# ldkong1205/OpenESS

Hardware: AMD Instinct MI355X
Metric: event-frames/sec fwd+bwd @640x480 B=8 (higher is better)
Workload: dtype bf16; 1 GPU; DSEC 640x480 5-bin x20 voxelizer + frame2voxel_pixel_distill pre-train step (E2VID-recurrent encoder x20, SemSegE2VID decoder, dilated-R50 teacher, Dice+CE), batch 8/GPU, random-init weights; global_batch=8, parallelism=dp1

## Files before the change

### openess_amd/csrc/conv5x5s2_halo.h

```cpp
constexpr int S2_PH = 8, S2_PW = 16;
constexpr int S2_HH = 2 * S2_PH + 3, S2_XW = 18;
constexpr int S2_BLOCKS = 2 * S2_HH * S2_XW;
constexpr int S2_HINSTR = (S2_BLOCKS + 63) / 64;
constexpr int S2_HALO_BYTES = S2_HINSTR * 4 * 1024;
constexpr int S2_SLAB = 64 * 64;
constexpr int S2_RING_PLAIN = 6, S2_RING_FUSED = 5;
constexpr int S2_LDS = S2_HALO_BYTES + S2_RING_PLAIN * S2_SLAB;
constexpr int S2_VH = S2_HH + 4, S2_VW = 2 * S2_PW + 3 + 4;
constexpr int S2_VINSTR = (S2_VH * S2_VW + 255) / 256;
constexpr int S2_VTOTAL = (S2_VH * S2_VW + 63) / 64;
constexpr int S2_VOX_BYTES = S2_VTOTAL * 1024;
constexpr int S2_LDS_FUSED = S2_HALO_BYTES + S2_RING_FUSED * S2_SLAB + S2_VOX_BYTES;
struct S2Head {
    const uint16_t* x8;
    long long x8_stride;
    const uint16_t* hw;
    const float* hb;
    int relu;
    const float* ev;
    int Ctot, c0, Cs, normalize;
    const double* stats;
};
constexpr int S2_IMG_PITCH = 72;

template <typename F, int... Is>
__device__ __forceinline__ void s2_for_taps(F&& f, std::integer_sequence<int, Is...>) { (f(std::integral_constant<int, Is>{}), ...); }

template <bool FUSED>
__device__ __forceinline__ void conv5x5s2_halo_tile(const ConvArgs& a, const S2Head& hd, const int bid, unsigned char* smem) {
    constexpr int S2_RING = FUSED ? S2_RING_FUSED : S2_RING_PLAIN;
    const int tile_n = bid % a.tiles_n;
    int patch = bid / a.tiles_n;
    const int tiles_x = (a.Wo + S2_PW - 1) / S2_PW, tiles_y = (a.Ho + S2_PH - 1) / S2_PH;
    const int ox0 = (patch % tiles_x) * S2_PW; patch /= tiles_x;
    const int oy0 = (patch % tiles_y) * S2_PH;
    const int b = patch / tiles_y;
    const int n0 = tile_n * 64;
    const int tid = threadIdx.x, lane = tid & 63;
    const int wave = __builtin_amdgcn_readfirstlane(tid >> 6);
    const int wm = wave >> 1, wn = wave & 1;
    constexpr int MT = 2, NT = 1;
    const int nchunks = a.Cin >> 5;
    const int NS = nchunks * 25;

    const long long in_bytes = FUSED ? (((long long)a.B * a.H * a.W - 1) * hd.x8_stride + 8) * 2
                                     : (((long long)a.B * a.H * a.W - 1) * a.in_pix_stride + a.Cin) * 2;
    __amdgpu_buffer_rsrc_t rsA = __builtin_amdgcn_make_buffer_rsrc(FUSED ? (void*)hd.x8 : (void*)a.in, 0, (FUSED && !hd.x8) ? 0 : (int)in_bytes, 0x00020000);
    __amdgpu_buffer_rsrc_t rsB = __builtin_amdgcn_make_buffer_rsrc((void*)a.w, 0, 0x7ffffff0, 0x00020000);

    unsigned hoff[FUSED ? 1 : S2_HINSTR];
#pragma unroll
    for (int i = 0; i < (FUSED ? 0 : S2_HINSTR); ++i) {
        const int u = (wave * S2_HINSTR + i) * 16 + (lane >> 2), slot = lane & 3;
        const int p = u / (S2_HH * S2_XW), rem = u - p * (S2_HH * S2_XW);
        const int hy = rem / S2_XW, xi = rem - hy * S2_XW;
        const int hx = 2 * xi + p;
        const int f = ((xi >> 2) & 1) | (((hy >> 1) & 1) << 1);
        const int iy = 2 * oy0 - 2 + hy, ix = 2 * ox0 - 2 + hx;
        const bool ok = u < S2_BLOCKS && hx < 2 * S2_PW + 3 && (unsigned)iy < (unsigned)a.H && (unsigned)ix < (unsigned)a.W;
        hoff[i] = ok ? (unsigned)((((long long)b * a.H + iy) * a.W + ix) * a.in_pix_stride * 2 + ((slot ^ f) << 4)) : 0x80000000u;
    }
    unsigned boff;
    {
        const int row = wave * 16 + (lane >> 2), slot = lane & 3;
        boff = (unsigned)(((n0 + row) * a.Kpad + ((slot ^ ((row >> 2) & 3)) << 3)) * 2);
    }
    auto issue_halo = [&](int cc) {
#pragma unroll
        for (int i = 0; i < (FUSED ? 0 : S2_HINSTR); ++i) {
            const unsigned voff = hoff[i] == 0x80000000u ? 0x80000000u : hoff[i] + (unsigned)(cc * 64);
            __builtin_amdgcn_raw_ptr_buffer_load_lds(rsA, (__attribute__((address_space(3))) void*)(smem + (wave * S2_HINSTR + i) * 1024),
                                                     16, voff, 0, 0, 0);
        }
    };
    auto issue_w = [&](int s, int buf) {
        const int cc = s / 25, tap = s - cc * 25;
        const unsigned voff = s < NS ? boff + (unsigned)((tap * a.Cin + cc * 32) * 2) : 0x80000000u;
        __builtin_amdgcn_raw_ptr_buffer_load_lds(rsB, (__attribute__((address_space(3))) void*)(smem + S2_HALO_BYTES + buf * S2_SLAB + wave * 1024),
                                                 16, voff, 0, 0, 0);
    };

    f32x16_t acc[2];
#pragma unroll
    for (int i = 0; i < 2; ++i)
#pragma unroll
        for (int e = 0; e < 16; ++e) acc[i][e] = 0.0f;

    const uint32_t lds0 = (uint32_t)(uintptr_t)smem;
    const int r31 = lane & 31, half = lane >> 5;
    const int a_px = (r31 & 7) + 8 * (r31 >> 4);
    uint32_t va[2][3][2], vb;
#pragma unroll
    for (int i = 0; i < 2; ++i) {
        const int py = 4 * wm + 2 * i + ((r31 >> 3) & 1);
#pragma unroll
        for (int sv = 0; sv < 3; ++sv)
#pragma unroll
            for (int rp = 0; rp < 2; ++rp) {
                const int f = (((a_px + sv) >> 2) & 1) | (((py + rp) & 1) << 1);
                va[i][sv][rp] = lds0 + (uint32_t)((2 * py * S2_XW + a_px) * 64 + ((half ^ f) << 4));
            }
    }
    {
        const int n = wn * 32 + r31;
        vb = lds0 + (uint32_t)(S2_HALO_BYTES + n * 64 + ((half ^ ((n >> 2) & 3)) << 4));
    }

#define S2_READ(FA, FB, R_, S_, KS_, BUF_)                                                                              \
    {                                                                                                                   \
        constexpr int blk_ = ((((S_) & 1) * S2_HH + (R_)) * S2_XW + ((S_) >> 1)) * 64;                                   \
        _Pragma("unroll") for (int i = 0; i < 2; ++i)                                                                   \
            asm volatile("ds_read_b128 %0, %1 offset:%2" : "=v"(FA[i]) : "v"(va[i][(S_) >> 1][((R_) >> 1) & 1] ^ (uint32_t)((KS_) << 5)), "n"(blk_) : "memory"); \
        asm volatile("ds_read_b128 %0, %1" : "=v"(FB[0]) : "v"((vb ^ (uint32_t)((KS_) << 5)) + (uint32_t)((BUF_) * S2_SLAB)) : "memory");  \
    }
#define S2_MMA(FA, FB)                                                                                                  \
    {                                                                                                                   \
        _Pragma("unroll") for (int i = 0; i < 2; ++i)                                                                   \
            acc[i] = __builtin_amdgcn_mfma_f32_32x32x16_bf16(FB[0], FA[i], acc[i], 0, 0, 0);                            \
    }

    if constexpr (FUSED) {
        unsigned char* vox = smem + S2_HALO_BYTES + S2_RING_FUSED * S2_SLAB;
        bf16x8_t wf[13];
        {
            const int p32 = lane & 31, hi = lane >> 5;
#pragma unroll
            for (int ks = 0; ks < 13; ++ks) wf[ks] = *reinterpret_cast<const bf16x8_t*>(hd.hw + (size_t)p32 * 256 + (ks * 2 + hi) * 8);
        }
        if (hd.ev) {
#pragma unroll
            for (int s = 0; s < S2_RING - 1; ++s) issue_w(s, s);
            const double nnz = hd.stats ? hd.stats[2] : 0.0;
            const bool active = hd.normalize && nnz > 0.0;
            float mean = 0.f, stdv = 1.f;
            if (active) {
                const float nf = (float)nnz;
                mean = (float)hd.stats[0] / nf;
                stdv = sqrtf(__fsub_rn((float)hd.stats[1] / nf, __fmul_rn(mean, mean)));
            }
            const long long hw_ = (long long)a.H * a.W;
            float raw[4][5];
            bool okv[4];
#pragma unroll
            for (int i = 0; i < 4; ++i) {
                const int v = tid + 256 * i;
                const int vy = v / S2_VW, vx = v - vy * S2_VW;
                const int iy = 2 * oy0 - 4 + vy, ix = 2 * ox0 - 4 + vx;
                okv[i] = v < S2_VH * S2_VW && (unsigned)iy < (unsigned)a.H && (unsigned)ix < (unsigned)a.W;
                const float* src = hd.ev + ((long long)b * hd.Ctot + hd.c0) * hw_ + (long long)iy * a.W + ix;
#pragma unroll
                for (int c = 0; c < 5; ++c) raw[i][c] = (okv[i] && c < hd.Cs) ? src[c * hw_] : 0.0f;
            }
#pragma unroll
            for (int i = 0; i < 4; ++i) {
                const int v = tid + 256 * i;
                float f[8] = {0.f, 0.f, 0.f, 0.f, 0.f, 0.f, 0.f, 0.f};
#pragma unroll
                for (int c = 0; c < 5; ++c) {
                    float q = raw[i][c];
                    if (active) q = __fmul_rn((q != 0.0f) ? 1.0f : 0.0f, __fsub_rn(q, mean)) / stdv;
                    f[c] = (okv[i] && c < hd.Cs) ? q : 0.0f;
                }
                const u32x4_t o = {pack_bf16x2(f[0], f[1]), pack_bf16x2(f[2], f[3]), pack_bf16x2(f[4], f[5]), pack_bf16x2(f[6], f[7])};
                if (v < S2_VTOTAL * 64)
                    asm volatile("ds_write_b128 %0, %1" :: "v"((uint32_t)(uintptr_t)vox + (uint32_t)(v * 16)), "v"(o) : "memory");
            }
            asm volatile("s_waitcnt lgkmcnt(0)" ::: "memory");
        } else {
#pragma unroll
            for (int i = 0; i < S2_VINSTR; ++i) {
                const int v = (wave * S2_VINSTR + i) * 64 + lane;
                const int vy = v / S2_VW, vx = v - vy * S2_VW;
                const int iy = 2 * oy0 - 4 + vy, ix = 2 * ox0 - 4 + vx;
                const bool ok = v < S2_VH * S2_VW && (unsigned)iy < (unsigned)a.H && (unsigned)ix < (unsigned)a.W;
                const unsigned voff = ok ? (unsigned)((((long long)b * a.H + iy) * a.W + ix) * hd.x8_stride * 2) : 0x80000000u;
                if (wave * S2_VINSTR + i < S2_VTOTAL)
                    __builtin_amdgcn_raw_ptr_buffer_load_lds(rsA, (__attribute__((address_space(3))) void*)(vox + (wave * S2_VINSTR + i) * 1024), 16, voff, 0, 0, 0);
            }
#pragma unroll
            for (int s = 0; s < S2_RING - 1; ++s) issue_w(s, s);
        }
        float bq[4][4];
#pragma unroll
        for (int q = 0; q < 4; ++q)
#pragma unroll
            for (int k = 0; k < 4; ++k) bq[q][k] = hd.hb ? hd.hb[8 * q + 4 * (lane >> 5) + k] : 0.0f;
        asm volatile("s_waitcnt vmcnt(0)" ::: "memory");
        __builtin_amdgcn_s_barrier();
        const uint32_t vox0 = (uint32_t)(uintptr_t)vox, pl0 = (uint32_t)(uintptr_t)smem;
        const int hi = lane >> 5;
        static_assert(((S2_BLOCKS + 31) / 32) % 2 == 0, "M-tiles are taken in pairs");
        for (int pr = wave; pr < (S2_BLOCKS + 31) / 64; pr += 4) {
            int uu_[2], hy_[2], xi_[2];
            bool inside_[2];
            uint32_t vbase[2];
#pragma unroll
            for (int z = 0; z < 2; ++z) {
                const int u = (2 * pr + z) * 32 + (lane & 31);
                uu_[z] = u;
                const int uu = u < S2_BLOCKS ? u : 0;
                const int p = uu / (S2_HH * S2_XW), rem = uu - p * (S2_HH * S2_XW);
                const int hy = rem / S2_XW, xi = rem - hy * S2_XW;
                int hx = 2 * xi + p;
                inside_[z] = u < S2_BLOCKS && hx < 2 * S2_PW + 3 && (unsigned)(2 * oy0 - 2 + hy) < (unsigned)a.H &&
                             (unsigned)(2 * ox0 - 2 + hx) < (unsigned)a.W;
                hx = hx < 2 * S2_PW + 3 ? hx : 0;
                hy_[z] = hy; xi_[z] = xi;
                vbase[z] = vox0 + (uint32_t)((hy * S2_VW + hx) * 16);
            }
            f32x16_t hacc[2];
#pragma unroll
            for (int z = 0; z < 2; ++z)
#pragma unroll
                for (int e = 0; e < 16; ++e) hacc[z][e] = 0.0f;
            bf16x8_t pa[2], pb[2];
#define S2_HREAD(DST, KS_)                                                                                             \
            {                                                                                                         \
                constexpr int t0_ = 2 * (KS_), t1_ = 2 * (KS_) + 1 < 25 ? 2 * (KS_) + 1 : 0;                            \
                const uint32_t off_ = hi ? (uint32_t)(((t1_ / 5) * S2_VW + t1_ % 5) * 16) : (uint32_t)(((t0_ / 5) * S2_VW + t0_ % 5) * 16); \
                asm volatile("ds_read_b128 %0, %1" : "=v"(DST[0]) : "v"(vbase[0] + off_) : "memory");                  \
                asm volatile("ds_read_b128 %0, %1" : "=v"(DST[1]) : "v"(vbase[1] + off_) : "memory");                  \
            }
            S2_HREAD(pa, 0)
            s2_for_taps([&](auto kc) __attribute__((always_inline)) {
                constexpr int ks = decltype(kc)::value;
                if constexpr (ks + 1 < 13) {
                    if constexpr (ks & 1) { S2_HREAD(pa, ks + 1) } else { S2_HREAD(pb, ks + 1) }
                    if constexpr (ks & 1) asm volatile("s_waitcnt lgkmcnt(2)" : "+v"(pb[0]), "+v"(pb[1]) :: "memory");
                    else asm volatile("s_waitcnt lgkmcnt(2)" : "+v"(pa[0]), "+v"(pa[1]) :: "memory");
                } else {
                    if constexpr (ks & 1) asm volatile("s_waitcnt lgkmcnt(0)" : "+v"(pb[0]), "+v"(pb[1]) :: "memory");
                    else asm volatile("s_waitcnt lgkmcnt(0)" : "+v"(pa[0]), "+v"(pa[1]) :: "memory");
                }
#pragma unroll
                for (int z = 0; z < 2; ++z)
                    hacc[z] = __builtin_amdgcn_mfma_f32_32x32x16_bf16(wf[ks], (ks & 1) ? pb[z] : pa[z], hacc[z], 0, 0, 0);
            }, std::make_integer_sequence<int, 13>{});
#undef S2_HREAD
#pragma unroll
            for (int z = 0; z < 2; ++z) {
                if (uu_[z] >= S2_BLOCKS) continue;
                const uint32_t f = (uint32_t)(((xi_[z] >> 2) & 1) | (((hy_[z] >> 1) & 1) << 1));
#pragma unroll
                for (int q = 0; q < 4; ++q) {
                    float v[4];
#pragma unroll
                    for (int k = 0; k < 4; ++k) {
                        v[k] = hacc[z][q * 4 + k] + bq[q][k];
                        if (hd.relu) v[k] = fmaxf(v[k], 0.0f);
                        v[k] = inside_[z] ? v[k] : 0.0f;
                    }
                    const uint2 o = make_uint2(pack_bf16x2(v[0], v[1]), pack_bf16x2(v[2], v[3]));
                    asm volatile("ds_write_b64 %0, %1" :: "v"(pl0 + (uint32_t)(uu_[z] * 64) + (((uint32_t)q ^ f) << 4) + (uint32_t)(8 * hi)), "v"(o) : "memory");
                }
            }
        }
        asm volatile("s_waitcnt lgkmcnt(0)" ::: "memory");
    } else {
#pragma unroll
        for (int s = 0; s < S2_RING - 1; ++s) issue_w(s, s);
    }
    int sg = 0, buf = 0;
    for (int cc = 0; cc < nchunks; ++cc) {
        if (cc > 0) __builtin_amdgcn_s_barrier();
        issue_halo(cc);
        asm volatile("s_waitcnt vmcnt(0)" ::: "memory");
        __builtin_amdgcn_s_barrier();
        bf16x8_t fa0[MT], fb0[NT], fa1[MT], fb1[NT];
        S2_READ(fa0, fb0, 0, 0, 0, buf)
        s2_for_taps([&](auto tc) __attribute__((always_inline)) {
            constexpr int t = decltype(tc)::value, r = t / 5, s = t - r * 5;
            if (t > 0) {
                asm volatile("s_waitcnt vmcnt(%0)" :: "n"(S2_RING - 3) : "memory");
                __builtin_amdgcn_s_barrier();
            }
            const int nb = buf + 1 == S2_RING ? 0 : buf + 1;
            issue_w(sg + S2_RING - 1, buf == 0 ? S2_RING - 1 : buf - 1);
            __builtin_amdgcn_s_setprio(3);
            S2_READ(fa1, fb1, r, s, 1, buf)
            OESS_FRAG_WAIT(3, fa0, fb0)
            S2_MMA(fa0, fb0)
            if constexpr (t < 24) {
                constexpr int r2 = (t + 1) / 5, s2 = (t + 1) - r2 * 5;
                S2_READ(fa0, fb0, r2, s2, 0, nb)
                OESS_FRAG_WAIT(3, fa1, fb1)
            } else {
                OESS_FRAG_WAIT(0, fa1, fb1)
            }
            S2_MMA(fa1, fb1)
            __builtin_amdgcn_s_setprio(0);
            ++sg; buf = nb;
        }, std::make_integer_sequence<int, 25>{});
    }
#undef S2_READ
#undef S2_MMA
    asm volatile("s_waitcnt vmcnt(0)" ::: "memory");
    __syncthreads();

    uint16_t* img = reinterpret_cast<uint16_t*>(smem);
    {
        float bq[4][4];
#pragma unroll
        for (int q = 0; q < 4; ++q)
#pragma unroll
            for (int k = 0; k < 4; ++k) bq[q][k] = a.bias ? a.bias[n0 + wn * 32 + 8 * q + 4 * half + k] : 0.0f;
#pragma unroll
        for (int i = 0; i < 2; ++i) {
            const int py = 4 * wm + 2 * i + ((r31 >> 3) & 1);
            uint16_t* dst = img + (py * S2_PW + a_px) * S2_IMG_PITCH + wn * 32 + 4 * half;
#pragma unroll
            for (int q = 0; q < 4; ++q) {
                float v[4];
#pragma unroll
                for (int k = 0; k < 4; ++k) {
                    v[k] = acc[i][q * 4 + k] + bq[q][k];
                    if (a.relu) v[k] = fmaxf(v[k], 0.0f);
                }
                uint2 o;
                o.x = pack_bf16x2(v[0], v[1]);
                o.y = pack_bf16x2(v[2], v[3]);
                *reinterpret_cast<uint2*>(dst + 8 * q) = o;
            }
        }
    }
    __syncthreads();
#pragma unroll
    for (int k = 0; k < 4; ++k) {
        const int idx = tid + k * 256, pl = idx >> 3, c = idx & 7;
        const int oy = oy0 + (pl >> 4), ox = ox0 + (pl & 15);
        if (oy < a.Ho && ox < a.Wo)
            out_store16(a.out + (((long long)b * a.Ho + oy) * a.Wo + ox) * a.out_pix_stride + n0 + c * 8,
                        *reinterpret_cast<const uint4*>(img + pl * S2_IMG_PITCH + c * 8));
    }
}

template <bool FUSED>
__global__ __launch_bounds__(256, 2) void conv5x5s2_halo_kernel(ConvArgs a, S2Head hd) {
    extern __shared__ __attribute__((aligned(16))) unsigned char smem[];
    const int nwg = a.tiles_m * a.tiles_n;
    int bid = blockIdx.x;
    {
        const int q = nwg >> 3, r = nwg & 7, xcd = bid & 7, idx = bid >> 3;
        bid = (xcd < r ? xcd * (q + 1) : r * (q + 1) + (xcd - r) * q) + idx;
    }
    conv5x5s2_halo_tile<FUSED>(a, hd, bid, smem);
}

struct S2Group {
    ConvArgs a[2];
    int start8[3];
};
__global__ __launch_bounds__(256, 2) void conv5x5s2_halo_group_kernel(S2Group g) {
    extern __shared__ __attribute__((aligned(16))) unsigned char smem[];
    const int xcd = blockIdx.x & 7, idx = blockIdx.x >> 3;
    const int p = idx >= g.start8[1] ? 1 : 0;
    const int li = idx - g.start8[p];
    const ConvArgs& a = g.a[p];
    const int nwg = a.tiles_m * a.tiles_n;
    const int q = nwg >> 3, r = nwg & 7;
    if (li >= q + (xcd < r ? 1 : 0)) return;
    conv5x5s2_halo_tile<false>(a, S2Head{}, (xcd < r ? xcd * (q + 1) : r * (q + 1) + (xcd - r) * q) + li, smem);
}
```

### openess_amd/csrc/conv_fwd.hip

```cpp
#include <hip/hip_runtime.h>
#include <stdint.h>
#include <stdlib.h>
#include <string.h>
#include <stdio.h>
#include <map>
#include <mutex>
#include <vector>
#include "oess.h"
#include "oess_common.h"

namespace {
#include <type_traits>
#include <utility>
using namespace oess;

#include "conv_args.h"
#include "conv_frag.h"
#include "conv_general.h"
#include "conv_dma.h"
#include "conv3x3_halo.h"
#pragma clang diagnostic push
#pragma clang diagnostic ignored "-Wunused-lambda-capture"
#include "conv_lstm_w128.h"
#include "conv_w128_gemm.h"
// ... 376 lines not shown
}

int oess_conv2d_fwd_route(int B, int H, int W, int Cin, int Cout, int R, int S, int stride, int pad, int dil, int has_bias,
                          int relu, int has_residual, int out_is_f32, int with_tile_stats, long long in_pix_stride,
                          long long out_pix_stride, long long res_pix_stride, int out_aligned16, size_t workspace_bytes) {
    ConvPlan p;
    const int rc = conv_plan(conv_call(B, H, W, Cin, Cout, R, S, stride, pad, dil, relu, has_bias, has_residual, out_is_f32, with_tile_stats,
                                       out_aligned16, in_pix_stride, out_pix_stride, res_pix_stride, workspace_bytes), &p);
    return rc == OESS_OK ? p.route : rc;
}

int oess_convlstm_fused_route(int B, int H, int W, int Cin, long long in_pix_stride, int C_hidden, int R, int S, int pad,
                              long long hidden_pix_stride) {
    ConvPlan p;
    const int rc = conv_plan(lstm_call(B, H, W, Cin, in_pix_stride, C_hidden, R, S, pad, hidden_pix_stride), &p);
    return rc == OESS_OK ? p.route : rc;
}

int oess_conv2d_route_count(void) { return OESS_ROUTE_COUNT; }

const char* oess_conv2d_route_name(int route) {
    static const char* const names[OESS_ROUTE_COUNT + 1] = {
        "?", "conv_smallcin_kernel<5, 5>", "conv_fwd_kernel<128>", "conv_fwd_kernel<64>", "conv_fwd_kernel<32>",
        "conv5x5s2_halo_kernel<false>", "conv_fwd_dma_kernel<128, 128, 4, true, 0, 512>", "conv3x3_w128_kernel",
        "conv3x3_halo_kernel<0>", "conv3x3_halo_kernel<1>", "conv_fwd_dma_kernel<128, 128, 2, true, 1>",
        "conv_fwd_dma_kernel<128, 128, 2, false, 1>", "split-K conv_fwd_dma_kernel<128, 128, 2, true> + splitk_reduce_kernel",
        "split-K conv_fwd_dma_kernel<128, 128, 2, false> + splitk_reduce_kernel", "conv1x1_w128_kernel",
        "conv_fwd_dma_kernel<256, 256, 2, true>", "conv_fwd_dma32_kernel<128, true, 0, 3>", "conv_fwd_dma_kernel<64, 128, 2, true>",
        "conv_fwd_dma_kernel<64, 128, 2, false>", "conv_fwd_dma_kernel<128, 128, 2, true>", "conv_fwd_dma_kernel<128, 128, 2, false>",
        "conv_fwd_dma_kernel<128, 64, 2, true>", "conv_fwd_dma_kernel<128, 64, 2, false>", "conv_fwd_dma_kernel<128, 32, 2, true>",
        "conv_fwd_dma_kernel<128, 32, 2, false>"};
    const int k = OESS_ROUTE_KERNEL(route);
    return route > 0 && k >= 1 && k <= OESS_ROUTE_COUNT ? names[k] : names[0];
}

int oess_convlstm_fused_bf16(const void* in, long long in_pix_stride, int B, int H, int W, int Cin, const void* w_packed_gates,
                             const float* bias, int C_hidden, int R, int S, int pad, const float* prev_cell, float* cell,
                             void* hidden, long long hidden_pix_stride, oess_stream_t stream) {
    if (!in || !hidden || !w_packed_gates || !cell) return OESS_EINVAL;
    {
        const char* i0 = (const char*)in; const char* i1 = i0 + ((long long)B * H * W - 1) * in_pix_stride * 2 + (long long)Cin * 2;
        const char* h0 = (const char*)hidden; const char* h1 = h0 + ((long long)B * H * W - 1) * hidden_pix_stride * 2 + (long long)C_hidden * 2;
        if (h0 < i1 && i0 < h1) return OESS_EINVAL;
    }
    ConvPlan p;
    const int rc = conv_plan(lstm_call(B, H, W, Cin, in_pix_stride, C_hidden, R, S, pad, hidden_pix_stride), &p);
    if (rc != OESS_OK) return rc;
    return conv_launch(p, ConvPtrs{in, w_packed_gates, bias, nullptr, nullptr, nullptr, nullptr, prev_cell, cell, hidden, nullptr}, stream);
}

int oess_convlstm_fused_group_bf16(const oess_convlstm_desc_t* d, int n, oess_stream_t stream) {
    if (!d || n <= 0 || n > 3) return OESS_EINVAL;
    for (int i = 0; i < n; ++i)
        if (!d[i].in || !d[i].hidden || !d[i].cell || d[i].B <= 0 || d[i].H <= 0 || d[i].W <= 0) return OESS_EINVAL;
    if (lstm_group_overlap(d, n, false)) return OESS_EINVAL;
    ConvArgs args[3];
    bool grouped = n >= 2;
    for (int i = 0; i < n && grouped; ++i) grouped = lstm_group_args(d[i], &args[i]);
    if (!grouped) {
        for (int i = 0; i < n; ++i) {
            const int rc = oess_convlstm_fused_bf16(d[i].in, d[i].in_pix_stride, d[i].B, d[i].H, d[i].W, d[i].Cin, d[i].w_packed_gates,
                                                    d[i].bias, d[i].C_hidden, d[i].R, d[i].S, d[i].pad, d[i].prev_cell, d[i].cell,
                                                    d[i].hidden, d[i].hidden_pix_stride, stream);
            if (rc != OESS_OK) return rc;
        }
        return OESS_OK;
    }
    conv_set_attrs();
    int order[3] = {0, 1, 2};
    for (int i = 1; i < n; ++i)
        for (int j = i; j > 0 && args[order[j]].Kpad > args[order[j - 1]].Kpad; --j) { const int t = order[j]; order[j] = order[j - 1]; order[j - 1] = t; }
    ConvGroup g;
    memset(&g, 0, sizeof(g));
    int at = 0;
    for (int i = 0; i < 3; ++i) {
        g.start8[i] = at;
        if (i < n) {
            g.a[i] = args[order[i]];
            at += (g.a[i].tiles_m * g.a[i].tiles_n + 7) / 8;
        }
    }
    g.start8[3] = at;
    static const int use256 = [] { const char* e = getenv("OESS_LSTM256"); return e ? atoi(e) : 1; }();
    if (use256) {
        ConvGroup big, small;
        memset(&big, 0, sizeof(big)); memset(&small, 0, sizeof(small));
        int nb = 0, ns = 0;
        for (int i = 0; i < n; ++i) {
            const ConvArgs& a = g.a[i];
            const bool fits = a.R == 3 && a.dil == 1 && (a.dil + 255 + a.dil * ((256 + a.W - 2) / a.W) + a.dil + 1) <= HALO_ROWS_256 &&
                              a.tiles_n * 128 == a.Cout;
            if (fits && (use256 == 1 || a.Kpad / BK >= 30)) big.a[nb++] = a; else small.a[ns++] = a;
        }
        auto layout = [](ConvGroup& q, int cnt, int rows) {
            int at_ = 0;
            for (int i = 0; i < 3; ++i) {
                q.start8[i] = at_;
                if (i < cnt) {
                    q.a[i].tiles_m = (q.a[i].M + rows - 1) / rows;
                    at_ += (q.a[i].tiles_m * q.a[i].tiles_n + 7) / 8;
                }
            }
            q.start8[3] = at_;
            return at_;
        };
        if (nb) {
            const int atb = layout(big, nb, 256);
            const size_t lds256 = (size_t)2 * HALO_ROWS_256 * 128 + (size_t)2 * 128 * 128;
            hipLaunchKernelGGL(conv3x3_halo256_group_kernel, dim3(8 * atb), dim3(512), lds256, (hipStream_t)stream, big);
        }
        if (ns) {
            const int ats = layout(small, ns, 128);
            const size_t lds128 = (size_t)2 * HALO_ROWS * 128 + (size_t)2 * 128 * 128;
            hipLaunchKernelGGL((conv3x3_halo_group_kernel<1>), dim3(8 * ats), dim3(CONV_THREADS), lds128, (hipStream_t)stream, small);
        }
        OESS_HIP(hipGetLastError());
        return OESS_OK;
    }
    const size_t lds = (size_t)2 * HALO_ROWS * 128 + (size_t)2 * 128 * 128;
    hipLaunchKernelGGL((conv3x3_halo_group_kernel<1>), dim3(8 * at), dim3(CONV_THREADS), lds, (hipStream_t)stream, g);
    OESS_HIP(hipGetLastError());
    return OESS_OK;
}

}

namespace {
struct W128Sched { int* dev; int stride; int grid; };
static int w128_tile_lists(const ConvArgs* a, int n, int grid, std::vector<int>* flat, int* stride_out) {
    if (grid < 8 || grid % 8) return OESS_EINVAL;
    const int per = grid / 8;
    std::vector<std::vector<int>> lists(grid);
    std::vector<long long> load(grid, 0);
    for (int x = 0; x < 8; ++x)
        for (int p = 0; p < n; ++p) {
            const int nwg = a[p].tiles_m * a[p].tiles_n, q = nwg >> 3, r = nwg & 7;
            const int cnt = q + (x < r ? 1 : 0), base = x < r ? x * (q + 1) : r * (q + 1) + (x - r) * q;
            const long long cost = (long long)(a[p].Cin / 64) * 9 * 2330 + 20000;
            for (int li = 0; li < cnt; ++li) {
                int best = 0;
                for (int c = 1; c < per; ++c) if (load[c * 8 + x] < load[best * 8 + x]) best = c;
                lists[best * 8 + x].push_back((p << 24) | (base + li));
                load[best * 8 + x] += cost;
            }
        }
    size_t longest = 0;
    for (auto& l : lists) longest = l.size() > longest ? l.size() : longest;
    if (longest > (size_t)W128_MAX_LIST) return OESS_EINVAL;
    const int stride = (int)longest + 1;
    flat->assign((size_t)grid * stride, -1);
    for (int b = 0; b < grid; ++b) for (size_t k = 0; k < lists[b].size(); ++k) (*flat)[(size_t)b * stride + k] = lists[b][k];
    *stride_out = stride;
    return OESS_OK;
}
static int w128_schedule(const ConvArgs* a, int n, W128Sched* out) {
    static std::mutex mu;
    static std::map<std::vector<int>, W128Sched> cache;
    std::vector<int> key;
    static const int grid_env = [] { const char* e = getenv("OESS_W128_GRID"); return e ? atoi(e) : 0; }();
    const int grid = (grid_env >= 8 && grid_env <= num_cus()) ? grid_env / 8 * 8 : num_cus();
    int dev = 0;
    (void)hipGetDevice(&dev);
    key.push_back(dev);
    key.push_back(grid);
    for (int i = 0; i < n; ++i) { key.push_back(a[i].tiles_m); key.push_back(a[i].tiles_n); key.push_back(a[i].Cin); }
    std::lock_guard<std::mutex> lk(mu);
    auto it = cache.find(key);
    if (it != cache.end()) { *out = it->second; return OESS_OK; }
    std::vector<int> flat;
    int stride = 0;
    if (w128_tile_lists(a, n, grid, &flat, &stride) != OESS_OK) return OESS_EINVAL;
    W128Sched sc{nullptr, stride, grid};
    if (hipMalloc((void**)&sc.dev, flat.size() * sizeof(int) + (size_t)grid * 4 * 16 * sizeof(float)) != hipSuccess) return OESS_ELAUNCH;
    if (hipMemcpy(sc.dev, flat.data(), flat.size() * sizeof(int), hipMemcpyHostToDevice) != hipSuccess) return OESS_ELAUNCH;
    cache[key] = sc;
    *out = sc;
    return OESS_OK;
}
}

extern "C" {
int oess_convlstm_w128_tile_lists(const int* tiles_m, const int* tiles_n, const int* cin, int n, int grid, int* lists, int capacity, int* stride) {
    if (!tiles_m || !tiles_n || !cin || !stride || n <= 0 || n > 3) return OESS_EINVAL;
    ConvArgs a[3];
    memset(a, 0, sizeof(a));
    for (int i = 0; i < n; ++i) { a[i].tiles_m = tiles_m[i]; a[i].tiles_n = tiles_n[i]; a[i].Cin = cin[i]; }
    std::vector<int> flat;
    const int rc = w128_tile_lists(a, n, grid, &flat, stride);
    if (rc != OESS_OK) return rc;
    if (lists) {
        if ((size_t)capacity < flat.size()) return OESS_ENOMEM;
        memcpy(lists, flat.data(), flat.size() * sizeof(int));
    }
    return OESS_OK;
}

size_t oess_convlstm_w128_cell_bytes(long long pixels, int C_hidden) {
    if (pixels <= 0 || C_hidden <= 0 || (C_hidden & 63)) return 0;
    return (size_t)((pixels + 255) / 256 * 256) * (size_t)C_hidden * 4;
}

int oess_convlstm_w128_cell_relayout(const float* src, float* dst, long long pixels, int C_hidden, int to_tiled, oess_stream_t stream) {
    if (!src || !dst || src == dst || pixels <= 0 || C_hidden <= 0 || (C_hidden & 63)) return OESS_EINVAL;
    const long long total = (pixels + 255) / 256 * 256 * C_hidden;
    long long blocks = (total + 255) / 256;
    if (blocks > 8192) blocks = 8192;
    hipLaunchKernelGGL(w128_cell_relayout_kernel, dim3((unsigned)blocks), dim3(256), 0, (hipStream_t)stream, src, dst, pixels, C_hidden, to_tiled);
    OESS_HIP(hipGetLastError());
    return OESS_OK;
}

int oess_convlstm_w128_group_bf16(const oess_convlstm_desc_t* d, int n, oess_stream_t stream) {
    if (!d || n <= 0 || n > 3) return OESS_EINVAL;
    int ctot = 0;
    for (int i = 0; i < n; ++i) {
        if (!d[i].in || !d[i].hidden || !d[i].cell || d[i].B <= 0 || d[i].H < 8 || d[i].W <= 0 || d[i].R != 3 || d[i].S != 3 || d[i].pad != 1 ||
            d[i].C_hidden <= 0 || (d[i].C_hidden & 63) || d[i].Cin <= 0 || (d[i].Cin & 63))
            return OESS_EINVAL;
        ctot += 4 * d[i].C_hidden;
        const long long px = (long long)d[i].B * d[i].H * d[i].W;
        const size_t cb = oess_convlstm_w128_cell_bytes(px, d[i].C_hidden);
        if (cb >= 0x7fffffffull || px * d[i].W >= 0x100000000ll) return OESS_EINVAL;
        if (d[i].prev_cell && d[i].prev_cell != d[i].cell) {
            const char *p0 = (const char*)d[i].prev_cell, *c0 = (const char*)d[i].cell;
            if (p0 < c0 + cb && c0 < p0 + cb) return OESS_EINVAL;
        }
        if ((px - 1) * d[i].hidden_pix_stride * 2 + (long long)d[i].C_hidden * 2 >= 0x7fffffffll) return OESS_EINVAL;
    }
    if (lstm_group_overlap(d, n, true)) return OESS_EINVAL;
    if (ctot > W128_BIAS_FLOATS) return OESS_EINVAL;
    ConvArgs args[3];
    for (int i = 0; i < n; ++i) {
        if (!lstm_group_args(d[i], &args[i])) return OESS_EINVAL;
        ConvArgs& a = args[i];
        if (a.Kpad != 9 * a.Cin || (1 + 255 + ((256 + a.W - 2) / a.W) + 1 + 1) > W128_HROWS || ((256 + a.W - 2) / a.W + 1) > a.H || !a.mg_w || !a.mg_wd)
            return OESS_EINVAL;
        a.tiles_m = (a.M + 255) / 256;
        a.tiles_n = a.Cout / 256;
    }
    conv_set_attrs();
    int order[3] = {0, 1, 2};
    for (int i = 1; i < n; ++i)
        for (int j = i; j > 0 && args[order[j]].Kpad > args[order[j - 1]].Kpad; --j) { const int t = order[j]; order[j] = order[j - 1]; order[j - 1] = t; }
    W128Group g;
    memset(&g, 0, sizeof(g));
    for (int i = 0; i < n; ++i) g.a[i] = args[order[i]];
    g.n = n;
    W128Sched sc;
    const int rc = w128_schedule(g.a, n, &sc);
    if (rc != OESS_OK) return rc;
    g.sched = sc.dev; g.sched_stride = sc.stride;
    hipLaunchKernelGGL(conv3x3_lstm_w128_kernel, dim3(sc.grid), dim3(256), (size_t)W128_LDS, (hipStream_t)stream, g);
    OESS_HIP(hipGetLastError());
#if (W128_ABL & 8192)
    {
        std::vector<float> st((size_t)sc.grid * 64);
        (void)hipDeviceSynchronize();
        (void)hipMemcpy(st.data(), sc.dev + (size_t)sc.grid * sc.stride, st.size() * 4, hipMemcpyDeviceToHost);
        double sum[16] = {0};
        for (int b = 0; b < sc.grid; ++b) for (int k = 0; k < 16; ++k) sum[k] += st[((size_t)b * 4) * 16 + k];
        fprintf(stderr, "w128 stamps (wave 0, cycles per workgroup, mean of %d): dx0 G0..G3 | dx1 | dx2 | setup+fill-issue  first-operand-wait  cell-update  tiles\n  ", sc.grid);
        double loop = 0;
        for (int k = 0; k < 12; ++k) { fprintf(stderr, "%9.0f%s", sum[k] / sc.grid, (k & 3) == 3 ? " |" : ""); loop += sum[k] / sc.grid; }
        fprintf(stderr, " %9.0f %9.0f %9.0f %5.1f   loop %9.0f\n", sum[12] / sc.grid, sum[13] / sc.grid, sum[14] / sc.grid, sum[15] / sc.grid, loop);
        double mn = 1e30, mx = 0, mean = 0;
        for (int b = 0; b < sc.grid; ++b) {
            double t = 0;
            for (int k = 0; k < 15; ++k) t += st[((size_t)b * 4) * 16 + k];
            mn = t < mn ? t : mn; mx = t > mx ? t : mx; mean += t / sc.grid;
        }
        fprintf(stderr, "  stamped cycles per workgroup: min %.0f mean %.0f max %.0f\n", mn, mean, mx);
    }
#endif
    return OESS_OK;
}
}

extern "C" {
int oess_conv5x5s2_group_bf16(const oess_conv_s2_desc_t* d, int n, oess_stream_t stream) {
    if (!d || n <= 0 || n > 2) return OESS_EINVAL;
    for (int i = 0; i < n; ++i)
        if (!d[i].in || !d[i].w_packed || !d[i].out || d[i].B <= 0 || d[i].H <= 0 || d[i].W <= 0) return OESS_EINVAL;
    if (n == 2) {
        const char *lo[2][2], *hi[2][2];
        long long st[2][2], cb[2][2];
        for (int i = 0; i < 2; ++i) {
            const long long pin = (long long)d[i].B * d[i].H * d[i].W;
            const long long pout = (long long)d[i].B * ((d[i].H - 1) / 2 + 1) * ((d[i].W - 1) / 2 + 1);
            st[i][0] = d[i].in_pix_stride * 2; cb[i][0] = (long long)d[i].Cin * 2;
            st[i][1] = d[i].out_pix_stride * 2; cb[i][1] = (long long)d[i].Cout * 2;
            lo[i][0] = (const char*)d[i].in; hi[i][0] = lo[i][0] + (pin - 1) * st[i][0] + cb[i][0];
            lo[i][1] = (const char*)d[i].out; hi[i][1] = lo[i][1] + (pout - 1) * st[i][1] + cb[i][1];
        }
        for (int i = 0; i < 2; ++i)
            for (int k = 0; k < 2; ++k) {
                if (!(lo[i][1] < hi[1 - i][k] && lo[1 - i][k] < hi[i][1])) continue;
                const long long S = st[i][1];
                if (S != st[1 - i][k] || S <= 0) return OESS_EINVAL;
                const long long diff = (long long)(lo[1 - i][k] - lo[i][1]);
                const long long delta = ((diff % S) + S) % S;
                if (!(delta >= cb[i][1] && delta + cb[1 - i][k] <= S)) return OESS_EINVAL;
            }
    }
    ConvPlan plan[2];
    ConvPtrs q[2];
    int rc[2];
    bool grouped = n == 2;
    for (int i = 0; i < n; ++i) {
        q[i] = ConvPtrs{d[i].in, d[i].w_packed, d[i].bias, nullptr, d[i].out, nullptr, nullptr, nullptr, nullptr, nullptr, nullptr};
        rc[i] = conv_plan(conv_call(d[i].B, d[i].H, d[i].W, d[i].Cin, d[i].Cout, 5, 5, 2, 2, 1, d[i].relu, d[i].bias, false, false, false,
                                    aligned16(d[i].out), d[i].in_pix_stride, d[i].out_pix_stride, 0, 0), &plan[i]);
        grouped = grouped && rc[i] == OESS_OK && plan[i].route == OESS_ROUTE_S2_HALO;
    }
    if (!grouped) {
        for (int i = 0; i < n; ++i) {
            const int r = rc[i] != OESS_OK ? rc[i] : conv_launch(plan[i], q[i], stream);
            if (r != OESS_OK) return r;
        }
        return OESS_OK;
    }
    conv_set_attrs();
    S2Group g;
    memset(&g, 0, sizeof(g));
    const int first = plan[1].args.Cin > plan[0].args.Cin ? 1 : 0;
    g.a[0] = conv_bind(plan[first], q[first]); g.a[1] = conv_bind(plan[1 - first], q[1 - first]);
    g.start8[0] = 0;
    g.start8[1] = (g.a[0].tiles_m * g.a[0].tiles_n + 7) / 8;
    g.start8[2] = g.start8[1] + (g.a[1].tiles_m * g.a[1].tiles_n + 7) / 8;
    hipLaunchKernelGGL(conv5x5s2_halo_group_kernel, dim3(8 * g.start8[2]), dim3(256), S2_LDS, (hipStream_t)stream, g);
    OESS_HIP(hipGetLastError());
    return OESS_OK;
}

static int e2vid_head_enc0_launch(const S2Head& hd, int B, int H, int W, const void* enc_w_packed, const float* enc_bias, int enc_relu,
                                  void* out, long long out_pix_stride, oess_stream_t stream) {
    conv_set_attrs();
    ConvArgs a;
    memset(&a, 0, sizeof(a));
    a.w = (const uint16_t*)enc_w_packed; a.bias = enc_bias; a.out = (uint16_t*)out; a.out_pix_stride = out_pix_stride;
    a.B = B; a.H = H; a.W = W; a.Cin = 32; a.Cout = 64; a.R = 5; a.S = 5; a.stride = 2; a.pad = 2; a.dil = 1;
    a.Ho = (H - 1) / 2 + 1; a.Wo = (W - 1) / 2 + 1;
    a.Kpad = (25 * 32 + BK - 1) / BK * BK;
    a.M = B * a.Ho * a.Wo; a.relu = enc_relu;
    a.tiles_n = 1;
    a.tiles_m = s2_tiles_m(B, a.Ho, a.Wo);
    hipLaunchKernelGGL((conv5x5s2_halo_kernel<true>), dim3(a.tiles_m), dim3(256), S2_LDS_FUSED, (hipStream_t)stream, a, hd);
    OESS_HIP(hipGetLastError());
    return OESS_OK;
}

int oess_e2vid_events_head_enc0_bf16(const float* events, int B, int Ctot, int c0, int Cs, int H, int W, const double* stats,
                                     int normalize, const void* head_w_packed, const float* head_bias, int head_relu,
                                     const void* enc_w_packed, const float* enc_bias, int enc_relu, void* out,
                                     long long out_pix_stride, oess_stream_t stream) {
    if (!events || !head_w_packed || !enc_w_packed || !out || B <= 0 || H <= 0 || W <= 0 || Ctot <= 0 || c0 < 0 || Cs <= 0 ||
        Cs > 5 || c0 + Cs > Ctot || (normalize && !stats) || (out_pix_stride & 7) || out_pix_stride < 64 || (((uintptr_t)out) & 15) ||
        (unsigned)head_relu > 1u || (unsigned)enc_relu > 1u)
        return OESS_EINVAL;
    S2Head hd{nullptr, 8, (const uint16_t*)head_w_packed, head_bias, head_relu, events, Ctot, c0, Cs, normalize, stats};
    return e2vid_head_enc0_launch(hd, B, H, W, enc_w_packed, enc_bias, enc_relu, out, out_pix_stride, stream);
}

int oess_e2vid_head_enc0_bf16(const void* x8, long long x8_pix_stride, int B, int H, int W, const void* head_w_packed,
                              const float* head_bias, int head_relu, const void* enc_w_packed, const float* enc_bias, int enc_relu,
                              void* out, long long out_pix_stride, oess_stream_t stream) {
    if (!x8 || !head_w_packed || !enc_w_packed || !out || B <= 0 || H <= 0 || W <= 0 || (x8_pix_stride & 7) || x8_pix_stride < 8 ||
        (out_pix_stride & 7) || out_pix_stride < 64 || (((uintptr_t)out) & 15) || (unsigned)head_relu > 1u || (unsigned)enc_relu > 1u)
        return OESS_EINVAL;
    if ((((long long)B * H * W - 1) * x8_pix_stride + 8) * 2 >= 0x7ffffff0ll) return OESS_EINVAL;
    S2Head hd{(const uint16_t*)x8, x8_pix_stride, (const uint16_t*)head_w_packed, head_bias, head_relu, nullptr, 0, 0, 0, 0, nullptr};
    return e2vid_head_enc0_launch(hd, B, H, W, enc_w_packed, enc_bias, enc_relu, out, out_pix_stride, stream);
}

}
```

Baseline: 225.1 event-frames/s.

## Add 128-channel-wide tiles to the 5x5 stride-2 halo conv kernel

Adds an NT=2 variant of the 5x5 s2 halo conv tile that computes 128 output channels per workgroup, reusing each loaded input halo across twice as many MFMAs. The weight ring shrinks to 4 stages of double-width slabs, and the epilogue staging image pitch widens to hold 128 channels. The grouped launcher picks wide tiles when Cout is a multiple of 128 (env-switchable, on by default) and now also routes single convs through the group kernel. The aim is to halve redundant halo loads and raise arithmetic intensity, at the cost of more accumulator registers, a shallower prefetch ring, and fewer workgroups.

```diff
diff --git a/openess_amd/csrc/conv5x5s2_halo.h b/openess_amd/csrc/conv5x5s2_halo.h
--- a/openess_amd/csrc/conv5x5s2_halo.h
+++ b/openess_amd/csrc/conv5x5s2_halo.h
@@ -6,6 +6,8 @@
 constexpr int S2_SLAB = 64 * 64;
 constexpr int S2_RING_PLAIN = 6, S2_RING_FUSED = 5;
 constexpr int S2_LDS = S2_HALO_BYTES + S2_RING_PLAIN * S2_SLAB;
+constexpr int S2_RING_WIDE = 4;
+constexpr int S2_LDS_WIDE = S2_HALO_BYTES + S2_RING_WIDE * 2 * S2_SLAB;
 constexpr int S2_VH = S2_HH + 4, S2_VW = 2 * S2_PW + 3 + 4;
 constexpr int S2_VINSTR = (S2_VH * S2_VW + 255) / 256;
 constexpr int S2_VTOTAL = (S2_VH * S2_VW + 63) / 64;
@@ -22,24 +24,28 @@
     const double* stats;
 };
 constexpr int S2_IMG_PITCH = 72;
+static_assert(128 * (128 + 8) * 2 <= S2_HALO_BYTES, "the wide epilogue image fits the halo region");
 
 template <typename F, int... Is>
 __device__ __forceinline__ void s2_for_taps(F&& f, std::integer_sequence<int, Is...>) { (f(std::integral_constant<int, Is>{}), ...); }
 
-template <bool FUSED>
+template <bool FUSED, int NT = 1>
 __device__ __forceinline__ void conv5x5s2_halo_tile(const ConvArgs& a, const S2Head& hd, const int bid, unsigned char* smem) {
-    constexpr int S2_RING = FUSED ? S2_RING_FUSED : S2_RING_PLAIN;
-    const int tile_n = bid % a.tiles_n;
-    int patch = bid / a.tiles_n;
+    static_assert(NT == 1 || (NT == 2 && !FUSED), "64- or 128-channel tiles; the fused head keeps 64");
+    constexpr int S2_RING = FUSED ? S2_RING_FUSED : (NT == 2 ? S2_RING_WIDE : S2_RING_PLAIN);
+    constexpr int SLAB = S2_SLAB * NT;
+    const int tiles_n = a.tiles_n / NT;
+    const int tile_n = bid % tiles_n;
+    int patch = bid / tiles_n;
     const int tiles_x = (a.Wo + S2_PW - 1) / S2_PW, tiles_y = (a.Ho + S2_PH - 1) / S2_PH;
     const int ox0 = (patch % tiles_x) * S2_PW; patch /= tiles_x;
     const int oy0 = (patch % tiles_y) * S2_PH;
     const int b = patch / tiles_y;
-    const int n0 = tile_n * 64;
+    const int n0 = tile_n * 64 * NT;
     const int tid = threadIdx.x, lane = tid & 63;
     const int wave = __builtin_amdgcn_readfirstlane(tid >> 6);
     const int wm = wave >> 1, wn = wave & 1;
-    constexpr int MT = 2, NT = 1;
+    constexpr int MT = 2;
     const int nchunks = a.Cin >> 5;
     const int NS = nchunks * 25;
 
@@ -60,10 +66,11 @@
         const bool ok = u < S2_BLOCKS && hx < 2 * S2_PW + 3 && (unsigned)iy < (unsigned)a.H && (unsigned)ix < (unsigned)a.W;
         hoff[i] = ok ? (unsigned)((((long long)b * a.H + iy) * a.W + ix) * a.in_pix_stride * 2 + ((slot ^ f) << 4)) : 0x80000000u;
     }
-    unsigned boff;
-    {
-        const int row = wave * 16 + (lane >> 2), slot = lane & 3;
-        boff = (unsigned)(((n0 + row) * a.Kpad + ((slot ^ ((row >> 2) & 3)) << 3)) * 2);
+    unsigned boff[NT];
+#pragma unroll
+    for (int k = 0; k < NT; ++k) {
+        const int row = (4 * k + wave) * 16 + (lane >> 2), slot = lane & 3;
+        boff[k] = (unsigned)(((n0 + row) * a.Kpad + ((slot ^ ((row >> 2) & 3)) << 3)) * 2);
     }
     auto issue_halo = [&](int cc) {
 #pragma unroll
@@ -75,16 +82,21 @@
     };
     auto issue_w = [&](int s, int buf) {
         const int cc = s / 25, tap = s - cc * 25;
-        const unsigned voff = s < NS ? boff + (unsigned)((tap * a.Cin + cc * 32) * 2) : 0x80000000u;
-        __builtin_amdgcn_raw_ptr_buffer_load_lds(rsB, (__attribute__((address_space(3))) void*)(smem + S2_HALO_BYTES + buf * S2_SLAB + wave * 1024),
-                                                 16, voff, 0, 0, 0);
+#pragma unroll
+        for (int k = 0; k < NT; ++k) {
+            const unsigned voff = s < NS ? boff[k] + (unsigned)((tap * a.Cin + cc * 32) * 2) : 0x80000000u;
+            __builtin_amdgcn_raw_ptr_buffer_load_lds(rsB, (__attribute__((address_space(3))) void*)(smem + S2_HALO_BYTES + buf * SLAB + (4 * k + wave) * 1024),
+                                                     16, voff, 0, 0, 0);
+        }
     };
 
-    f32x16_t acc[2];
-#pragma unroll
-    for (int i = 0; i < 2; ++i)
-#pragma unroll
-        for (int e = 0; e < 16; ++e) acc[i][e] = 0.0f;
+    f32x16_t acc[MT][NT];
+#pragma unroll
+    for (int i = 0; i < MT; ++i)
+#pragma unroll
+        for (int j = 0; j < NT; ++j)
+#pragma unroll
+            for (int e = 0; e < 16; ++e) acc[i][j][e] = 0.0f;
 
     const uint32_t lds0 = (uint32_t)(uintptr_t)smem;
     const int r31 = lane & 31, half = lane >> 5;
@@ -102,7 +114,7 @@
             }
     }
     {
-        const int n = wn * 32 + r31;
+        const int n = wn * 32 * NT + r31;
         vb = lds0 + (uint32_t)(S2_HALO_BYTES + n * 64 + ((half ^ ((n >> 2) & 3)) << 4));
     }
 
@@ -111,12 +123,15 @@
         constexpr int blk_ = ((((S_) & 1) * S2_HH + (R_)) * S2_XW + ((S_) >> 1)) * 64;                                   \
         _Pragma("unroll") for (int i = 0; i < 2; ++i)                                                                   \
             asm volatile("ds_read_b128 %0, %1 offset:%2" : "=v"(FA[i]) : "v"(va[i][(S_) >> 1][((R_) >> 1) & 1] ^ (uint32_t)((KS_) << 5)), "n"(blk_) : "memory"); \
-        asm volatile("ds_read_b128 %0, %1" : "=v"(FB[0]) : "v"((vb ^ (uint32_t)((KS_) << 5)) + (uint32_t)((BUF_) * S2_SLAB)) : "memory");  \
+        asm volatile("ds_read_b128 %0, %1" : "=v"(FB[0]) : "v"((vb ^ (uint32_t)((KS_) << 5)) + (uint32_t)((BUF_) * SLAB)) : "memory");  \
+        if constexpr (NT == 2)                                                                                          \
+            asm volatile("ds_read_b128 %0, %1 offset:2048" : "=v"(FB[NT - 1]) : "v"((vb ^ (uint32_t)((KS_) << 5)) + (uint32_t)((BUF_) * SLAB)) : "memory"); \
     }
 #define S2_MMA(FA, FB)                                                                                                  \
     {                                                                                                                   \
-        _Pragma("unroll") for (int i = 0; i < 2; ++i)                                                                   \
-            acc[i] = __builtin_amdgcn_mfma_f32_32x32x16_bf16(FB[0], FA[i], acc[i], 0, 0, 0);                            \
+        _Pragma("unroll") for (int i = 0; i < MT; ++i)                                                                  \
+            _Pragma("unroll") for (int j = 0; j < NT; ++j)                                                              \
+                acc[i][j] = __builtin_amdgcn_mfma_f32_32x32x16_bf16(FB[j], FA[i], acc[i][j], 0, 0, 0);                  \
     }
 
     if constexpr (FUSED) {
@@ -271,19 +286,19 @@
         s2_for_taps([&](auto tc) __attribute__((always_inline)) {
             constexpr int t = decltype(tc)::value, r = t / 5, s = t - r * 5;
             if (t > 0) {
-                asm volatile("s_waitcnt vmcnt(%0)" :: "n"(S2_RING - 3) : "memory");
+                asm volatile("s_waitcnt vmcnt(%0)" :: "n"(NT * (S2_RING - 3)) : "memory");
                 __builtin_amdgcn_s_barrier();
             }
             const int nb = buf + 1 == S2_RING ? 0 : buf + 1;
             issue_w(sg + S2_RING - 1, buf == 0 ? S2_RING - 1 : buf - 1);
             __builtin_amdgcn_s_setprio(3);
             S2_READ(fa1, fb1, r, s, 1, buf)
-            OESS_FRAG_WAIT(3, fa0, fb0)
+            OESS_FRAG_WAIT(MT + NT, fa0, fb0)
             S2_MMA(fa0, fb0)
             if constexpr (t < 24) {
                 constexpr int r2 = (t + 1) / 5, s2 = (t + 1) - r2 * 5;
                 S2_READ(fa0, fb0, r2, s2, 0, nb)
-                OESS_FRAG_WAIT(3, fa1, fb1)
+                OESS_FRAG_WAIT(MT + NT, fa1, fb1)
             } else {
                 OESS_FRAG_WAIT(0, fa1, fb1)
             }
@@ -297,40 +312,45 @@
     asm volatile("s_waitcnt vmcnt(0)" ::: "memory");
     __syncthreads();
 
+    constexpr int PITCH = S2_IMG_PITCH + 64 * (NT - 1);
     uint16_t* img = reinterpret_cast<uint16_t*>(smem);
     {
-        float bq[4][4];
-#pragma unroll
-        for (int q = 0; q < 4; ++q)
-#pragma unroll
-            for (int k = 0; k < 4; ++k) bq[q][k] = a.bias ? a.bias[n0 + wn * 32 + 8 * q + 4 * half + k] : 0.0f;
-#pragma unroll
-        for (int i = 0; i < 2; ++i) {
+        float bq[NT][4][4];
+#pragma unroll
+        for (int j = 0; j < NT; ++j)
+#pragma unroll
+            for (int q = 0; q < 4; ++q)
+#pragma unroll
+                for (int k = 0; k < 4; ++k) bq[j][q][k] = a.bias ? a.bias[n0 + wn * 32 * NT + 32 * j + 8 * q + 4 * half + k] : 0.0f;
+#pragma unroll
+        for (int i = 0; i < MT; ++i) {
             const int py = 4 * wm + 2 * i + ((r31 >> 3) & 1);
-            uint16_t* dst = img + (py * S2_PW + a_px) * S2_IMG_PITCH + wn * 32 + 4 * half;
-#pragma unroll
-            for (int q = 0; q < 4; ++q) {
-                float v[4];
-#pragma unroll
-                for (int k = 0; k < 4; ++k) {
-                    v[k] = acc[i][q * 4 + k] + bq[q][k];
-                    if (a.relu) v[k] = fmaxf(v[k], 0.0f);
+            uint16_t* dst = img + (py * S2_PW + a_px) * PITCH + wn * 32 * NT + 4 * half;
+#pragma unroll
+            for (int j = 0; j < NT; ++j)
+#pragma unroll
+                for (int q = 0; q < 4; ++q) {
+                    float v[4];
+#pragma unroll
+                    for (int k = 0; k < 4; ++k) {
+                        v[k] = acc[i][j][q * 4 + k] + bq[j][q][k];
+                        if (a.relu) v[k] = fmaxf(v[k], 0.0f);
+                    }
+                    uint2 o;
+                    o.x = pack_bf16x2(v[0], v[1]);
+                    o.y = pack_bf16x2(v[2], v[3]);
+                    *reinterpret_cast<uint2*>(dst + 32 * j + 8 * q) = o;
                 }
-                uint2 o;
-                o.x = pack_bf16x2(v[0], v[1]);
-                o.y = pack_bf16x2(v[2], v[3]);
-                *reinterpret_cast<uint2*>(dst + 8 * q) = o;
-            }
         }
     }
     __syncthreads();
 #pragma unroll
-    for (int k = 0; k < 4; ++k) {
-        const int idx = tid + k * 256, pl = idx >> 3, c = idx & 7;
+    for (int k = 0; k < 4 * NT; ++k) {
+        const int idx = tid + k * 256, pl = idx / (8 * NT), c = idx % (8 * NT);
         const int oy = oy0 + (pl >> 4), ox = ox0 + (pl & 15);
         if (oy < a.Ho && ox < a.Wo)
             out_store16(a.out + (((long long)b * a.Ho + oy) * a.Wo + ox) * a.out_pix_stride + n0 + c * 8,
-                        *reinterpret_cast<const uint4*>(img + pl * S2_IMG_PITCH + c * 8));
+                        *reinterpret_cast<const uint4*>(img + pl * PITCH + c * 8));
     }
 }
 
@@ -348,6 +368,7 @@
 
 struct S2Group {
     ConvArgs a[2];
+    int wide[2], cnt[2];
     int start8[3];
 };
 __global__ __launch_bounds__(256, 2) void conv5x5s2_halo_group_kernel(S2Group g) {
@@ -356,8 +377,10 @@
     const int p = idx >= g.start8[1] ? 1 : 0;
     const int li = idx - g.start8[p];
     const ConvArgs& a = g.a[p];
-    const int nwg = a.tiles_m * a.tiles_n;
+    const int nwg = g.cnt[p];
     const int q = nwg >> 3, r = nwg & 7;
     if (li >= q + (xcd < r ? 1 : 0)) return;
-    conv5x5s2_halo_tile<false>(a, S2Head{}, (xcd < r ? xcd * (q + 1) : r * (q + 1) + (xcd - r) * q) + li, smem);
+    const int t = (xcd < r ? xcd * (q + 1) : r * (q + 1) + (xcd - r) * q) + li;
+    if (g.wide[p]) conv5x5s2_halo_tile<false, 2>(a, S2Head{}, t, smem);
+    else conv5x5s2_halo_tile<false, 1>(a, S2Head{}, t, smem);
 }
diff --git a/openess_amd/csrc/conv_fwd.hip b/openess_amd/csrc/conv_fwd.hip
--- a/openess_amd/csrc/conv_fwd.hip
+++ b/openess_amd/csrc/conv_fwd.hip
@@ -702,16 +702,21 @@
                 if (!(delta >= cb[i][1] && delta + cb[1 - i][k] <= S)) return OESS_EINVAL;
             }
     }
+    const char* wide_env = getenv("OESS_S2_WIDE");
+    const bool use_wide = wide_env ? atoi(wide_env) != 0 : true;
     ConvPlan plan[2];
     ConvPtrs q[2];
     int rc[2];
-    bool grouped = n == 2;
+    bool grouped = true, any_wide = false, wide_ok[2] = {false, false};
     for (int i = 0; i < n; ++i) {
         q[i] = ConvPtrs{d[i].in, d[i].w_packed, d[i].bias, nullptr, d[i].out, nullptr, nullptr, nullptr, nullptr, nullptr, nullptr};
         rc[i] = conv_plan(conv_call(d[i].B, d[i].H, d[i].W, d[i].Cin, d[i].Cout, 5, 5, 2, 2, 1, d[i].relu, d[i].bias, false, false, false,
                                     aligned16(d[i].out), d[i].in_pix_stride, d[i].out_pix_stride, 0, 0), &plan[i]);
         grouped = grouped && rc[i] == OESS_OK && plan[i].route == OESS_ROUTE_S2_HALO;
-    }
+        wide_ok[i] = use_wide && grouped && d[i].Cout % 128 == 0;
+        any_wide = any_wide || wide_ok[i];
+    }
+    if (n == 1 && !any_wide) grouped = false;
     if (!grouped) {
         for (int i = 0; i < n; ++i) {
             const int r = rc[i] != OESS_OK ? rc[i] : conv_launch(plan[i], q[i], stream);
@@ -722,12 +727,18 @@
     conv_set_attrs();
     S2Group g;
     memset(&g, 0, sizeof(g));
-    const int first = plan[1].args.Cin > plan[0].args.Cin ? 1 : 0;
-    g.a[0] = conv_bind(plan[first], q[first]); g.a[1] = conv_bind(plan[1 - first], q[1 - first]);
+    const int first = (n == 2 && plan[1].args.Cin > plan[0].args.Cin) ? 1 : 0;
+    bool wide[2] = {wide_ok[first], false};
+    g.a[0] = conv_bind(plan[first], q[first]);
+    if (n == 2) { g.a[1] = conv_bind(plan[1 - first], q[1 - first]); wide[1] = wide_ok[1 - first]; }
+    for (int p = 0; p < n; ++p) {
+        g.wide[p] = wide[p] ? 1 : 0;
+        g.cnt[p] = g.a[p].tiles_m * g.a[p].tiles_n / (wide[p] ? 2 : 1);
+    }
     g.start8[0] = 0;
-    g.start8[1] = (g.a[0].tiles_m * g.a[0].tiles_n + 7) / 8;
-    g.start8[2] = g.start8[1] + (g.a[1].tiles_m * g.a[1].tiles_n + 7) / 8;
-    hipLaunchKernelGGL(conv5x5s2_halo_group_kernel, dim3(8 * g.start8[2]), dim3(256), S2_LDS, (hipStream_t)stream, g);
+    g.start8[1] = (g.cnt[0] + 7) / 8;
+    g.start8[2] = g.start8[1] + (g.cnt[1] + 7) / 8;
+    hipLaunchKernelGGL(conv5x5s2_halo_group_kernel, dim3(8 * g.start8[2]), dim3(256), any_wide ? S2_LDS_WIDE : S2_LDS, (hipStream_t)stream, g);
     OESS_HIP(hipGetLastError());
     return OESS_OK;
 }
```

New measurement: 226.9 event-frames/s, median of 6. About the same (+0.8%).
